# anenbergb/Co-DETR-TensorRT

Hardware: AMD Instinct MI355X
Metric: images/sec, Co-DINO Swin-L 1920x1280 fp16 (p50 ms/image alongside) (higher is better)
Workload: dtype f16

## Files before the change

co-detr-tensorrt_amd/csrc/device_prims.h:

```cpp
#pragma once
#include <hip/hip_runtime.h>
#include <stdint.h>

namespace {

typedef _Float16 f16x8 __attribute__((ext_vector_type(8)));
typedef _Float16 f16x4 __attribute__((ext_vector_type(4)));
typedef _Float16 f16x2 __attribute__((ext_vector_type(2)));
typedef __bf16 bf16x8 __attribute__((ext_vector_type(8)));
typedef __bf16 bf16x4 __attribute__((ext_vector_type(4)));
typedef __bf16 bf16x2 __attribute__((ext_vector_type(2)));
typedef short s16x8 __attribute__((ext_vector_type(8)));
typedef short s16x4 __attribute__((ext_vector_type(4)));
typedef unsigned short u16x8 __attribute__((ext_vector_type(8)));
typedef unsigned short u16x4 __attribute__((ext_vector_type(4)));
typedef unsigned short u16x2 __attribute__((ext_vector_type(2)));
typedef float f32x4 __attribute__((ext_vector_type(4)));
typedef float f32x2 __attribute__((ext_vector_type(2)));
typedef unsigned u32x4 __attribute__((ext_vector_type(4)));
typedef unsigned u32x2 __attribute__((ext_vector_type(2)));
typedef int i32x8 __attribute__((ext_vector_type(8)));
typedef int i32x4 __attribute__((ext_vector_type(4)));

__device__ __forceinline__ float bf16_to_f32(unsigned short bits) { return __uint_as_float(((unsigned)bits) << 16); }
__device__ __forceinline__ unsigned short bf16_from_f32(float v) {
  const unsigned u = __float_as_uint(v);
  if ((u & 0x7fffffffu) > 0x7f800000u) return (unsigned short)((u >> 16) | 0x40);
  return (unsigned short)((u + 0x7fffu + ((u >> 16) & 1u)) >> 16);
}

template <class F, short kNegInf>
__device__ __forceinline__ F relu_bits16(F x) {
  s16x8 i;
  __builtin_memcpy(&i, &x, 16);
  u32x4 keep = __builtin_bit_cast(u32x4, __builtin_elementwise_sub_sat((s16x8)kNegInf, i) >> 15);
  asm("" : "+v"(keep));
  i = __builtin_bit_cast(s16x8, __builtin_bit_cast(u32x4, i) & keep);
  __builtin_memcpy(&x, &i, 16);
  return x;
}

struct HalfT {
  using elem = _Float16;
  using frag = f16x8;
  using v4 = f16x4;
  __device__ static f32x4 mfma(frag a, frag b, f32x4 c) { return __builtin_amdgcn_mfma_f32_16x16x32_f16(a, b, c, 0, 0, 0); }
  __device__ static float to_f32(unsigned short bits) {
    _Float16 h;
    __builtin_memcpy(&h, &bits, 2);
    return (float)h;
  }
  __device__ static unsigned short from_f32(float v) {
    _Float16 h = (_Float16)v;
    unsigned short bits;
    __builtin_memcpy(&bits, &h, 2);
    return bits;
  }
  __device__ static unsigned pack2(float lo, float hi) {
    f16x2 h = {(_Float16)lo, (_Float16)hi};
    unsigned o;
    __builtin_memcpy(&o, &h, 4);
    return o;
  }
  __device__ static s16x4 pack4(const float (&v)[4]) {
    f16x4 h = {(_Float16)v[0], (_Float16)v[1], (_Float16)v[2], (_Float16)v[3]};
    s16x4 o;
    __builtin_memcpy(&o, &h, 8);
    return o;
  }
  __device__ static frag relu(frag x) { return relu_bits16<frag, (short)0xfc00>(x); }
};
struct BFloatT {
  using elem = __bf16;
  using frag = bf16x8;
  using v4 = bf16x4;
  __device__ static f32x4 mfma(frag a, frag b, f32x4 c) { return __builtin_amdgcn_mfma_f32_16x16x32_bf16(a, b, c, 0, 0, 0); }
  __device__ static float to_f32(unsigned short bits) { return bf16_to_f32(bits); }
  __device__ static unsigned short from_f32(float v) {
    const __bf16 h = (__bf16)v;
    return __builtin_bit_cast(unsigned short, h);
  }
  __device__ static unsigned pack2(float lo, float hi) {
    const bf16x2 h = {(__bf16)lo, (__bf16)hi};
    return __builtin_bit_cast(unsigned, h);
  }
  __device__ static s16x4 pack4(const float (&v)[4]) {
    const bf16x4 h = {(__bf16)v[0], (__bf16)v[1], (__bf16)v[2], (__bf16)v[3]};
    return __builtin_bit_cast(s16x4, h);
  }
  __device__ static frag relu(frag x) { return relu_bits16<frag, (short)0xff80>(x); }
};

__device__ __forceinline__ float gelu_erf(float x) {
  const float u = fabsf(x);
  const float t = __builtin_amdgcn_rcpf(fmaf(0.3275911f * 0.70710678118654752f, u, 1.0f));
  float p = fmaf(0.5f * 1.061405429f, t, 0.5f * -1.453152027f);
  p = fmaf(p, t, 0.5f * 1.421413741f);
  p = fmaf(p, t, 0.5f * -0.284496736f);
  p = fmaf(p, t, 0.5f * 0.254829592f);
  const float ez = __builtin_amdgcn_exp2f(u * u * (-0.5f * 1.4426950408889634f));
  return fmaf(u, fmaf(-(p * t), ez, 0.5f), 0.5f * x);
}
__device__ __forceinline__ f32x2 gelu_erf2(f32x2 x) {
  const f32x2 u = {fabsf(x.x), fabsf(x.y)};
  const f32x2 d = __builtin_elementwise_fma(f32x2{0.3275911f * 0.70710678118654752f, 0.3275911f * 0.70710678118654752f}, u,
                                            f32x2{1.0f, 1.0f});
  const f32x2 t = {__builtin_amdgcn_rcpf(d.x), __builtin_amdgcn_rcpf(d.y)};
  f32x2 p = __builtin_elementwise_fma(f32x2{0.5f * 1.061405429f, 0.5f * 1.061405429f}, t,
                                      f32x2{0.5f * -1.453152027f, 0.5f * -1.453152027f});
  p = __builtin_elementwise_fma(p, t, f32x2{0.5f * 1.421413741f, 0.5f * 1.421413741f});
  p = __builtin_elementwise_fma(p, t, f32x2{0.5f * -0.284496736f, 0.5f * -0.284496736f});
  p = __builtin_elementwise_fma(p, t, f32x2{0.5f * 0.254829592f, 0.5f * 0.254829592f});
  const f32x2 e = (u * u) * f32x2{-0.5f * 1.4426950408889634f, -0.5f * 1.4426950408889634f};
  const f32x2 ez = {__builtin_amdgcn_exp2f(e.x), __builtin_amdgcn_exp2f(e.y)};
  const f32x2 h = __builtin_elementwise_fma(-(p * t), ez, f32x2{0.5f, 0.5f});
  return __builtin_elementwise_fma(u, h, x * f32x2{0.5f, 0.5f});
}

__device__ __forceinline__ unsigned xcd_tile(unsigned bid, unsigned nblk) {
  const unsigned q = nblk >> 3, r = nblk & 7u, x = bid & 7u, i = bid >> 3;
  return (x < r ? x * (q + 1) : r * (q + 1) + (x - r) * q) + i;
}

__device__ __forceinline__ void lds_dma16(const unsigned char* src, unsigned voff, unsigned lds_addr) {
  asm volatile("s_mov_b32 m0, %2\n\ts_nop 0\n\tglobal_load_lds_dwordx4 %0, %1" ::"v"(voff), "s"(src), "s"(lds_addr)
               : "memory", "m0");
}
__device__ __forceinline__ void lds_dma16(const unsigned char* src, unsigned voff, unsigned char* dst) {
  lds_dma16(src, voff, (unsigned)(uintptr_t)((__attribute__((address_space(3))) unsigned char*)dst));
}
__device__ __forceinline__ void lds_dma16_auto(const void* g, unsigned char* l) {
  __builtin_amdgcn_global_load_lds((const __attribute__((address_space(1))) void*)g,
                                   (__attribute__((address_space(3))) void*)l, 16, 0, 0);
}
template <int N>
__device__ __forceinline__ void wait_vmcnt() {
  asm volatile("s_waitcnt vmcnt(%0)" ::"n"(N) : "memory");
}

__device__ __forceinline__ int floor_i(float v) {
  int d;
  asm("v_cvt_flr_i32_f32 %0, %1" : "=v"(d) : "v"(v));
  return d;
}

template <int CTRL>
__device__ __forceinline__ unsigned dpp_u(unsigned v) {
  return (unsigned)__builtin_amdgcn_update_dpp(0, (int)v, CTRL, 0xf, 0xf, true);
}
template <int CTRL>
__device__ __forceinline__ float dpp_f(float v) {
  return __uint_as_float(dpp_u<CTRL>(__float_as_uint(v)));
}
constexpr int kXor1 = 0xB1, kXor2 = 0x4E;
__device__ __forceinline__ unsigned quad_bcast_u(unsigned v, int owner) {
  switch (owner) {
    case 0: return dpp_u<0x00>(v);
    case 1: return dpp_u<0x55>(v);
    case 2: return dpp_u<0xAA>(v);
    default: return dpp_u<0xFF>(v);
  }
}
__device__ __forceinline__ float quad_bcast_f(float v, int owner) { return __uint_as_float(quad_bcast_u(__float_as_uint(v), owner)); }
__device__ __forceinline__ unsigned quad_bcast_add(unsigned v, int owner, unsigned add) {
  unsigned d;
  switch (owner) {
    case 0: asm("v_add_u32_dpp %0, %1, %2 quad_perm:[0,0,0,0] row_mask:0xf bank_mask:0xf" : "=v"(d) : "v"(v), "v"(add)); break;
    case 1: asm("v_add_u32_dpp %0, %1, %2 quad_perm:[1,1,1,1] row_mask:0xf bank_mask:0xf" : "=v"(d) : "v"(v), "v"(add)); break;
    case 2: asm("v_add_u32_dpp %0, %1, %2 quad_perm:[2,2,2,2] row_mask:0xf bank_mask:0xf" : "=v"(d) : "v"(v), "v"(add)); break;
    default: asm("v_add_u32_dpp %0, %1, %2 quad_perm:[3,3,3,3] row_mask:0xf bank_mask:0xf" : "=v"(d) : "v"(v), "v"(add)); break;
  }
  return d;
}

}
```

co-detr-tensorrt_amd/csrc/ffn_fused.hip:

```cpp
#include <hip/hip_runtime.h>
#include <stdint.h>

#include <type_traits>

#include "codetr_hip.h"
#include "device_prims.h"
#include "large_lds.h"

#ifdef CODETR_FFN_ABL
#define CODETR_FFN_ABL_MASK CODETR_FFN_ABL
#else
#define CODETR_FFN_ABL_MASK 0
#endif
namespace {

constexpr int C = 256;
constexpr int BH = 64;
constexpr int kThreads = 256;
constexpr int kW1Bytes = BH * C * 2;
constexpr int kW2Bytes = C * BH * 2;
constexpr int kStageBytes = kW1Bytes + kW2Bytes;
constexpr int kMaxHidden = 8192;


template <class ET, int MTT = 2, bool OPROJ = false>
__global__ __launch_bounds__(kThreads) __attribute__((amdgpu_waves_per_eu(1, 1))) void ffn_fused_kernel(
    const unsigned short* __restrict__ X, const unsigned short* __restrict__ W1, const unsigned short* __restrict__ b1,
    const unsigned short* __restrict__ W2, const unsigned short* __restrict__ b2, unsigned short* __restrict__ Y, int M,
    int Hd, const unsigned short* __restrict__ ln_g, const unsigned short* __restrict__ ln_b, float ln_eps,
    const unsigned short* __restrict__ pos, unsigned short* __restrict__ Y2,
    const unsigned short* __restrict__ lnin_g, const unsigned short* __restrict__ lnin_b, float lnin_eps, int ntiles,
    const unsigned short* __restrict__ Wo = nullptr, const unsigned short* __restrict__ bo = nullptr,
    const unsigned short* __restrict__ ID = nullptr) {
  __shared__ __attribute__((aligned(16))) unsigned char lds[2 * kStageBytes + kMaxHidden * 2 + 2048];
  using E = typename ET::elem;
  using V8 = typename ET::frag;
  using V4 = typename ET::v4;
  constexpr int MT = MTT, WR = 16 * MT, TR = 4 * WR;
  const int tid = threadIdx.x, lane = tid & 63;
  const int wave = __builtin_amdgcn_readfirstlane(tid >> 6);
  const int l15 = lane & 15, grp = lane >> 4;
  const int nchunks = Hd / BH;
  unsigned char* ringA = lds;
  unsigned char* ringB = lds + 2 * kW1Bytes;
  unsigned short* sB1 = reinterpret_cast<unsigned short*>(lds + 2 * kStageBytes);
  unsigned short* sLn = reinterpret_cast<unsigned short*>(lds + 2 * kStageBytes + kMaxHidden * 2);
  unsigned short* sB2 = sLn + 512;
  unsigned short* sBo = sB2 + 256;

  unsigned w1_voff[2];
#pragma unroll
  for (int par = 0; par < 2; ++par)
    w1_voff[par] = (unsigned)((tid >> 5) * (C * 2) + (((tid & 31) ^ ((par * 8 + (tid >> 5)) & 15)) * 16));
  const unsigned w2_voff = (unsigned)((tid >> 3) * Hd * 2 + (((tid & 7) ^ ((tid >> 4) & 7)) * 16));
  const unsigned char* W1b = reinterpret_cast<const unsigned char*>(W1);
  const unsigned char* W2b = reinterpret_cast<const unsigned char*>(W2);
  const unsigned char* Wob = reinterpret_cast<const unsigned char*>(Wo);
  auto stage_w1 = [&](int p, int c, unsigned char* dst) {
    lds_dma16(W1b + (size_t)c * kW1Bytes + p * 4096, w1_voff[p & 1], dst + (p * kThreads + wave * 64) * 16);
  };
  auto stage_wo = [&](int p, int c, unsigned char* dst) {
    lds_dma16(Wob + (size_t)c * kW1Bytes + p * 4096, w1_voff[p & 1], dst + (p * kThreads + wave * 64) * 16);
  };
  auto stage_w2 = [&](int q, int c, unsigned char* dst) {
    lds_dma16(W2b + (size_t)q * 64 * Hd + c * (BH * 2), w2_voff, dst + (q * kThreads + wave * 64) * 16);
  };
#pragma unroll
  for (int p = 0; p < 8; ++p) {
    if (OPROJ) stage_wo(p, 0, ringA);
    else stage_w1(p, 0, ringA);
  }
#pragma unroll
  for (int p = 0; p < 8; ++p) stage_w2(p, 0, ringB);
  if (OPROJ) {
#pragma unroll
    for (int p = 0; p < 8; ++p) stage_wo(p, 1, ringA + kW1Bytes);
  }

  V8 xn[MT][8];
  auto load_x = [&](int tile, int mt) {
    int m = tile * TR + wave * WR + mt * 16 + l15;
    m = m < M ? m : M - 1;
#pragma unroll
    for (int ks = 0; ks < 8; ++ks) xn[mt][ks] = *reinterpret_cast<const V8*>(X + (size_t)m * C + ks * 32 + grp * 8);
  };
#pragma unroll
  for (int mt = 0; mt < MT; ++mt) load_x(blockIdx.x, mt);
  for (int i = tid; i < Hd / 8; i += kThreads)
    *reinterpret_cast<s16x8*>(sB1 + i * 8) = *reinterpret_cast<const s16x8*>(b1 + i * 8);
  if (ln_g && tid < 64) {
    const int i = tid & 31;
    *reinterpret_cast<s16x8*>(sLn + (tid >> 5) * 256 + i * 8) = *reinterpret_cast<const s16x8*>((tid >> 5 ? ln_b : ln_g) + i * 8);
  }
  if (tid >= 64 && tid < 96) *reinterpret_cast<s16x8*>(sB2 + (tid - 64) * 8) = *reinterpret_cast<const s16x8*>(b2 + (tid - 64) * 8);
  if (OPROJ && tid >= 96 && tid < 128) *reinterpret_cast<s16x8*>(sBo + (tid - 96) * 8) = *reinterpret_cast<const s16x8*>(bo + (tid - 96) * 8);
  asm volatile("s_waitcnt lgkmcnt(0)" ::: "memory");

  int gc = 0;
  int ga = 0;
  for (int tile = blockIdx.x; tile < ntiles; tile += gridDim.x) {
    const int m0 = tile * TR + wave * WR;
    V8 xf[MT][8];
    f32x4 yacc[16][MT];
    if constexpr (OPROJ) {
      const int cb = 16 * (grp & 1) + 8 * (grp >> 1);
      V8 idn[MT][8];
#pragma unroll
      for (int mt = 0; mt < MT; ++mt) {
        int m = m0 + mt * 16 + l15;
        m = m < M ? m : M - 1;
#pragma unroll
        for (int j = 0; j < 8; ++j) {
          if (CODETR_FFN_ABL_MASK & 32) idn[mt][j] = xn[mt][j];
          else idn[mt][j] = *reinterpret_cast<const V8*>(ID + (size_t)m * C + 32 * j + cb);
        }
      }
#pragma unroll
      for (int mt = 0; mt < MT; ++mt) asm volatile("" ::"v"(xn[mt][7]) : "memory");
#pragma unroll
      for (int nt = 0; nt < 16; ++nt)
#pragma unroll
        for (int mt = 0; mt < MT; ++mt) yacc[nt][mt] = f32x4{0.f, 0.f, 0.f, 0.f};
      unsigned char* const A0 = ringA + (ga & 1) * kW1Bytes;
      unsigned char* const A1 = ringA + ((ga + 1) & 1) * kW1Bytes;
      unsigned char* const B1 = ringB + ((gc + 1) & 1) * kW2Bytes;
#pragma unroll
      for (int pc = 0; pc < 4; ++pc) {
        const unsigned char* sW = pc == 0 ? A0 : pc == 1 ? A1 : pc == 2 ? B1 : A0;
        if (pc >= 2 && !(CODETR_FFN_ABL_MASK & 256)) wait_vmcnt<8>();
        __builtin_amdgcn_s_barrier();
        auto read_wo = [&](int ks, V8 (&a)[4]) {
#pragma unroll
          for (int ht = 0; ht < 4; ++ht) {
            const int row = ht * 16 + l15;
            const int chunk = (ks * 4 + grp) ^ (row & 15);
            a[ht] = *reinterpret_cast<const V8*>(sW + row * (C * 2) + chunk * 16);
          }
        };
        V8 aw[2][4];
        read_wo(0, aw[0]);
#pragma unroll
        for (int ks = 0; ks < 8; ++ks) {
          if (ks + 1 < 8) read_wo(ks + 1, aw[(ks + 1) & 1]);
          if (pc == 0 && !(CODETR_FFN_ABL_MASK & 256)) stage_wo(ks, 2, B1);
          else if (pc == 1 && !(CODETR_FFN_ABL_MASK & 256)) stage_wo(ks, 3, A0);
          else if (pc == 2) stage_w1(ks, 0, A1);
#pragma unroll
          for (int i = 0; i < 4 * MT; ++i)
            if (!(CODETR_FFN_ABL_MASK & 128))
              yacc[4 * pc + i / MT][i % MT] = ET::mfma(aw[ks & 1][i / MT], xn[i % MT][ks], yacc[4 * pc + i / MT][i % MT]);
            else asm volatile("" ::"v"(aw[ks & 1][i / MT]));
          __builtin_amdgcn_sched_group_barrier(0x008, 2, 0);
          __builtin_amdgcn_sched_group_barrier(0x100, 4, 0);
          __builtin_amdgcn_sched_group_barrier(0x008, 4 * MT - 2, 0);
          __builtin_amdgcn_sched_barrier(0);
        }
      }
      ga += 3;
      const int oddp = grp & 1;
      if (CODETR_FFN_ABL_MASK & 64) {
#pragma unroll
        for (int mt = 0; mt < MT; ++mt)
#pragma unroll
          for (int j = 0; j < 8; ++j) {
            xf[mt][j] = xn[mt][j];
            asm volatile("" ::"v"(idn[mt][j]), "v"(yacc[2 * j][mt]), "v"(yacc[2 * j + 1][mt]));
          }
      } else
#pragma unroll
      for (int mt = 0; mt < MT; ++mt) {
        unsigned yp[16][2];
#pragma unroll
        for (int nt = 0; nt < 16; ++nt) {
          const V4 bb = *reinterpret_cast<const V4*>(sBo + nt * 16 + grp * 4);
          const V4 y = {(E)(yacc[nt][mt][0] + (float)bb[0]), (E)(yacc[nt][mt][1] + (float)bb[1]),
                        (E)(yacc[nt][mt][2] + (float)bb[2]), (E)(yacc[nt][mt][3] + (float)bb[3])};
          __builtin_memcpy(yp[nt], &y, 8);
        }
        float o[8][8];
        float sm = 0.f;
#pragma unroll
        for (int j = 0; j < 8; ++j) {
          const unsigned s0 = oddp ? yp[2 * j][0] : yp[2 * j + 1][0], s1 = oddp ? yp[2 * j][1] : yp[2 * j + 1][1];
          const unsigned k0 = oddp ? yp[2 * j + 1][0] : yp[2 * j][0], k1 = oddp ? yp[2 * j + 1][1] : yp[2 * j][1];
          const unsigned r0 = (unsigned)__shfl_xor((int)s0, 16, 64), r1 = (unsigned)__shfl_xor((int)s1, 16, 64);
          const unsigned z[4] = {oddp ? r0 : k0, oddp ? r1 : k1, oddp ? k0 : r0, oddp ? k1 : r1};
          V8 yv;
          __builtin_memcpy(&yv, z, 16);
#pragma unroll
          for (int e = 0; e < 8; ++e) {
            o[j][e] = (float)(E)((float)yv[e] + (float)idn[mt][j][e]);
            sm += o[j][e];
          }
        }
        if (lnin_g) {
          sm += __shfl_xor(sm, 16, 64);
          sm += __shfl_xor(sm, 32, 64);
          const float mean = sm * (1.0f / C);
          float q = 0.f;
#pragma unroll
          for (int j = 0; j < 8; ++j)
#pragma unroll
            for (int e = 0; e < 8; ++e) {
              const float d = o[j][e] - mean;
              q = fmaf(d, d, q);
            }
          q += __shfl_xor(q, 16, 64);
          q += __shfl_xor(q, 32, 64);
          const float rstd = rsqrtf(q * (1.0f / C) + lnin_eps);
#pragma unroll
          for (int j = 0; j < 8; ++j) {
            const V8 gw = *reinterpret_cast<const V8*>(lnin_g + 32 * j + cb);
            const V8 gb = *reinterpret_cast<const V8*>(lnin_b + 32 * j + cb);
#pragma unroll
            for (int e = 0; e < 8; ++e) o[j][e] = fmaf((o[j][e] - mean) * rstd, (float)gw[e], (float)gb[e]);
          }
        }
#pragma unroll
        for (int j = 0; j < 8; ++j)
#pragma unroll
          for (int e = 0; e < 8; ++e) xf[mt][j][e] = (E)o[j][e];
      }
    } else {
#pragma unroll
    for (int mt = 0; mt < MT; ++mt) {
      if (lnin_g) {
        float sm = 0.f;
#pragma unroll
        for (int ks = 0; ks < 8; ++ks)
#pragma unroll
          for (int e = 0; e < 8; ++e) sm += (float)xn[mt][ks][e];
        sm += __shfl_xor(sm, 16, 64);
        sm += __shfl_xor(sm, 32, 64);
        const float mean = sm * (1.0f / C);
        float q = 0.f;
#pragma unroll
        for (int ks = 0; ks < 8; ++ks)
#pragma unroll
          for (int e = 0; e < 8; ++e) {
            const float d = (float)xn[mt][ks][e] - mean;
            q = fmaf(d, d, q);
          }
        q += __shfl_xor(q, 16, 64);
        q += __shfl_xor(q, 32, 64);
        const float rstd = rsqrtf(q * (1.0f / C) + lnin_eps);
#pragma unroll
        for (int ks = 0; ks < 8; ++ks) {
          const V8 gw = *reinterpret_cast<const V8*>(lnin_g + ks * 32 + grp * 8);
          const V8 gb = *reinterpret_cast<const V8*>(lnin_b + ks * 32 + grp * 8);
#pragma unroll
          for (int e = 0; e < 8; ++e)
            xf[mt][ks][e] = (E)fmaf(((float)xn[mt][ks][e] - mean) * rstd, (float)gw[e], (float)gb[e]);
        }
      } else {
#pragma unroll
        for (int ks = 0; ks < 8; ++ks) xf[mt][ks] = xn[mt][ks];
      }
      asm volatile("" ::"v"(xn[mt][7]) : "memory");
    }
    }
#pragma unroll
    for (int nt = 0; nt < 16; ++nt)
#pragma unroll
      for (int mt = 0; mt < MT; ++mt) yacc[nt][mt] = f32x4{0.f, 0.f, 0.f, 0.f};

    for (int c = 0; c < nchunks; ++c, ++gc, ++ga) {
      const int cn = c + 1 < nchunks ? c + 1 : 0;
      const unsigned char* sW1 = ringA + (ga & 1) * kW1Bytes;
      const unsigned char* sW2 = ringB + (gc & 1) * kW2Bytes;
      unsigned char* nW1 = ringA + ((ga + 1) & 1) * kW1Bytes;
      unsigned char* nW2 = ringB + ((gc + 1) & 1) * kW2Bytes;
      const unsigned char* nsrc1 = (OPROJ && c + 1 == nchunks) ? Wob : W1b + (size_t)cn * kW1Bytes;
      if (!(CODETR_FFN_ABL_MASK & 8)) {
        if (c > 0) wait_vmcnt<8>();
        else if (OPROJ) wait_vmcnt<0>();
        __builtin_amdgcn_s_barrier();
      }

      f32x4 hacc[4][MT];
#pragma unroll
      for (int ht = 0; ht < 4; ++ht) {
        const V4 bv = *reinterpret_cast<const V4*>(sB1 + c * BH + ht * 16 + grp * 4);
        const f32x4 b4 = {(float)bv[0], (float)bv[1], (float)bv[2], (float)bv[3]};
#pragma unroll
        for (int mt = 0; mt < MT; ++mt) hacc[ht][mt] = b4;
      }
      auto read_w1 = [&](int ks, V8 (&a)[4]) {
#pragma unroll
        for (int ht = 0; ht < 4; ++ht) {
          const int row = ht * 16 + l15;
          const int chunk = (ks * 4 + grp) ^ (row & 15);
          a[ht] = *reinterpret_cast<const V8*>(sW1 + row * (C * 2) + chunk * 16);
        }
      };
      V8 aw[2][4];
      read_w1(0, aw[0]);
#pragma unroll
      for (int ks = 0; ks < 8; ++ks) {
        if (ks + 1 < 8 && !(CODETR_FFN_ABL_MASK & 4)) read_w1(ks + 1, aw[(ks + 1) & 1]);
        if (!(CODETR_FFN_ABL_MASK & 1)) lds_dma16(nsrc1 + ks * 4096, w1_voff[ks & 1], nW1 + (ks * kThreads + wave * 64) * 16);
#pragma unroll
        for (int i = 0; i < 4 * MT; ++i)
          if (!(CODETR_FFN_ABL_MASK & 2))
            hacc[i / MT][i % MT] = ET::mfma(aw[(CODETR_FFN_ABL_MASK & 4) ? 0 : (ks & 1)][i / MT], xf[i % MT][ks], hacc[i / MT][i % MT]);
          else if (!(CODETR_FFN_ABL_MASK & 4)) asm volatile("" ::"v"(aw[ks & 1][i / MT]));
        __builtin_amdgcn_sched_group_barrier(0x008, 2, 0);
        __builtin_amdgcn_sched_group_barrier(0x100, 4, 0);
        __builtin_amdgcn_sched_group_barrier(0x008, 4 * MT - 2, 0);
        __builtin_amdgcn_sched_barrier(0);
      }
      V8 pf[2][MT];
      if (CODETR_FFN_ABL_MASK & 16) {
#pragma unroll
        for (int s = 0; s < 2; ++s)
#pragma unroll
          for (int mt = 0; mt < MT; ++mt) pf[s][mt] = xf[mt][s];
#pragma unroll
        for (int ht = 0; ht < 4; ++ht)
#pragma unroll
          for (int mt = 0; mt < MT; ++mt) asm volatile("" ::"v"(hacc[ht][mt]));
      } else
#pragma unroll
      for (int s = 0; s < 2; ++s)
#pragma unroll
        for (int mt = 0; mt < MT; ++mt)
#pragma unroll
          for (int h = 0; h < 2; ++h)
#pragma unroll
            for (int r = 0; r < 4; ++r) pf[s][mt][h * 4 + r] = (E)hacc[2 * s + h][mt][r];
      if (!(CODETR_FFN_ABL_MASK & 16))
#pragma unroll
      for (int s = 0; s < 2; ++s)
#pragma unroll
        for (int mt = 0; mt < MT; ++mt) pf[s][mt] = ET::relu(pf[s][mt]);
      if (!(CODETR_FFN_ABL_MASK & 8)) {
        if (c > 0) wait_vmcnt<8>();
        __builtin_amdgcn_s_barrier();
      }
      auto read_w2 = [&](int ntp, V8 (&a)[4]) {
#pragma unroll
        for (int t = 0; t < 2; ++t) {
          const int n = (2 * ntp + t) * 16 + l15;
          const unsigned char* rowp = sW2 + n * (BH * 2);
          const int sw = (n >> 1) & 7;
#pragma unroll
          for (int s = 0; s < 2; ++s) a[t * 2 + s] = *reinterpret_cast<const V8*>(rowp + ((4 * s + grp) ^ sw) * 16);
        }
      };
      V8 a2[2][4];
      read_w2(0, a2[0]);
#pragma unroll
      for (int ntp = 0; ntp < 8; ++ntp) {
        if (ntp + 1 < 8 && !(CODETR_FFN_ABL_MASK & 4)) read_w2(ntp + 1, a2[(ntp + 1) & 1]);
        if (!(CODETR_FFN_ABL_MASK & 1)) stage_w2(ntp, cn, nW2);
#pragma unroll
        for (int i = 0; i < 4 * MT; ++i) {
          const int ts = i / MT, mt = i % MT, nt = 2 * ntp + ts / 2;
          if (!(CODETR_FFN_ABL_MASK & 2))
            yacc[nt][mt] = ET::mfma(a2[(CODETR_FFN_ABL_MASK & 4) ? 0 : (ntp & 1)][ts], pf[ts & 1][mt], yacc[nt][mt]);
          else if (!(CODETR_FFN_ABL_MASK & 4)) asm volatile("" ::"v"(a2[ntp & 1][ts]));
        }
        __builtin_amdgcn_sched_group_barrier(0x008, 2, 0);
        __builtin_amdgcn_sched_group_barrier(0x100, 4, 0);
        __builtin_amdgcn_sched_group_barrier(0x008, 4 * MT - 2, 0);
        __builtin_amdgcn_sched_barrier(0);
      }
    }

    const int next_tile = tile + (int)gridDim.x < ntiles ? tile + (int)gridDim.x : tile;
    if (OPROJ) {
#pragma unroll
      for (int p = 0; p < 8; ++p) stage_wo(p, 1, ringA + ((ga + 1) & 1) * kW1Bytes);
    }
    const int odd = grp & 1;
    const int cbase = 16 * odd + 8 * (grp >> 1);
    const int src_lane4 = (l15 + 16 * (2 * odd + (grp >> 1))) * 4;
#pragma unroll
    for (int mt = 0; mt < MT; ++mt) {
      const int m = m0 + mt * 16 + l15;
      if (MT == 2 && mt == 0) load_x(next_tile, 0);
      unsigned yp[16][2];
#pragma unroll
      for (int nt = 0; nt < 16; ++nt) {
        const V4 bb = *reinterpret_cast<const V4*>(sB2 + nt * 16 + grp * 4);
        const V4 y = {(E)(yacc[nt][mt][0] + (float)bb[0]), (E)(yacc[nt][mt][1] + (float)bb[1]),
                      (E)(yacc[nt][mt][2] + (float)bb[2]), (E)(yacc[nt][mt][3] + (float)bb[3])};
        __builtin_memcpy(yp[nt], &y, 8);
      }
      float o[8][8];
      float sm = 0.f;
#pragma unroll
      for (int j = 0; j < 8; ++j) {
        const unsigned s0 = odd ? yp[2 * j][0] : yp[2 * j + 1][0], s1 = odd ? yp[2 * j][1] : yp[2 * j + 1][1];
        const unsigned k0 = odd ? yp[2 * j + 1][0] : yp[2 * j][0], k1 = odd ? yp[2 * j + 1][1] : yp[2 * j][1];
        const unsigned r0 = (unsigned)__shfl_xor((int)s0, 16, 64), r1 = (unsigned)__shfl_xor((int)s1, 16, 64);
        const unsigned z[4] = {odd ? r0 : k0, odd ? r1 : k1, odd ? k0 : r0, odd ? k1 : r1};
        V8 yv, xid;
        __builtin_memcpy(&yv, z, 16);
        int xw[4];
        __builtin_memcpy(xw, &xf[mt][j], 16);
        if (!OPROJ)
#pragma unroll
        for (int d = 0; d < 4; ++d) xw[d] = __builtin_amdgcn_ds_bpermute(src_lane4, xw[d]);
        __builtin_memcpy(&xid, xw, 16);
#pragma unroll
        for (int e = 0; e < 8; ++e) {
          o[j][e] = (float)(E)((float)yv[e] + (float)xid[e]);
          sm += o[j][e];
        }
      }
      V8 pr[8];
      if (Y2) {
        const unsigned short* prow = pos + (size_t)(m < M ? m : M - 1) * C + cbase;
#pragma unroll
        for (int j = 0; j < 8; ++j) pr[j] = *reinterpret_cast<const V8*>(prow + 32 * j);
      }
      if (mt == 0) load_x(next_tile, MT - 1);
      if (ln_g) {
        sm += __shfl_xor(sm, 16, 64);
        sm += __shfl_xor(sm, 32, 64);
        const float mean = sm * (1.0f / C);
        float q = 0.f;
#pragma unroll
        for (int j = 0; j < 8; ++j)
#pragma unroll
          for (int e = 0; e < 8; ++e) {
            const float d = o[j][e] - mean;
            q = fmaf(d, d, q);
          }
        q += __shfl_xor(q, 16, 64);
        q += __shfl_xor(q, 32, 64);
        const float rstd = rsqrtf(q * (1.0f / C) + ln_eps);
#pragma unroll
        for (int j = 0; j < 8; ++j) {
          const V8 gw = *reinterpret_cast<const V8*>(sLn + 32 * j + cbase);
          const V8 gb = *reinterpret_cast<const V8*>(sLn + 256 + 32 * j + cbase);
#pragma unroll
          for (int e = 0; e < 8; ++e) o[j][e] = (float)(E)fmaf((o[j][e] - mean) * rstd, (float)gw[e], (float)gb[e]);
        }
      }
      if (m < M) {
        unsigned short* yrow = Y + (size_t)m * C + cbase;
#pragma unroll
        for (int j = 0; j < 8; ++j) {
          V8 ov;
#pragma unroll
          for (int e = 0; e < 8; ++e) ov[e] = (E)o[j][e];
          *reinterpret_cast<V8*>(yrow + 32 * j) = ov;
        }
        if (Y2) {
          unsigned short* y2row = Y2 + (size_t)m * C + cbase;
#pragma unroll
          for (int j = 0; j < 8; ++j) {
            V8 ov;
#pragma unroll
            for (int e = 0; e < 8; ++e) ov[e] = (E)(o[j][e] + (float)pr[j][e]);
            *reinterpret_cast<V8*>(y2row + 32 * j) = ov;
          }
        }
      }
    }
  }
  wait_vmcnt<0>();
}

__global__ void pack_w2_kernel(const unsigned short* __restrict__ w2, unsigned short* __restrict__ out, int64_t total) {
  const int64_t i = (int64_t)blockIdx.x * blockDim.x + threadIdx.x;
  if (i >= total) return;
  const int col = (int)(i & 63);
  const int s = col >> 5, g = (col >> 3) & 3, j = col & 7;
  const int old = 32 * s + (j < 4 ? 4 * g + j : 16 + 4 * g + (j - 4));
  out[i] = w2[(i & ~(int64_t)63) + old];
}

}

namespace {

template <class ET>
int ffn_entry(void* stream, const void* x_dev, const void* w1_dev, const void* b1_dev,
                            const void* w2_packed_dev, const void* b2_dev, void* y_dev, int64_t M, int64_t C_in,
                            int64_t hidden, const void* ln_in_gamma_dev, const void* ln_in_beta_dev, float ln_in_eps,
                            const void* ln_gamma_dev, const void* ln_beta_dev, float ln_eps, const void* pos_dev,
                            void* y_plus_pos_dev, const void* wo_dev = nullptr, const void* bo_dev = nullptr,
                            const void* identity_dev = nullptr) {
  const void* w2_dev = w2_packed_dev;
  if (!x_dev || !w1_dev || !b1_dev || !w2_dev || !b2_dev || !y_dev || M <= 0 || hidden <= 0) return CODETR_E_BADARG;
  const bool oproj = wo_dev != nullptr;
  if (oproj && (!bo_dev || !identity_dev)) return CODETR_E_BADARG;
  if ((reinterpret_cast<uintptr_t>(wo_dev) | reinterpret_cast<uintptr_t>(bo_dev) | reinterpret_cast<uintptr_t>(identity_dev)) & 15)
    return CODETR_E_BADARG;
  if ((ln_gamma_dev == nullptr) != (ln_beta_dev == nullptr) || (pos_dev == nullptr) != (y_plus_pos_dev == nullptr) ||
      (ln_in_gamma_dev == nullptr) != (ln_in_beta_dev == nullptr))
    return CODETR_E_BADARG;
  if (C_in != C || hidden % BH != 0 || hidden > kMaxHidden) return CODETR_E_UNSUPPORTED;
  if (M > 0x7fffffffLL - 256 || hidden > 0x7fffffffLL) return CODETR_E_TOO_LARGE;
  if ((reinterpret_cast<uintptr_t>(x_dev) | reinterpret_cast<uintptr_t>(w1_dev) | reinterpret_cast<uintptr_t>(b1_dev) |
       reinterpret_cast<uintptr_t>(w2_dev) | reinterpret_cast<uintptr_t>(b2_dev) | reinterpret_cast<uintptr_t>(y_dev) |
       reinterpret_cast<uintptr_t>(ln_in_gamma_dev) | reinterpret_cast<uintptr_t>(ln_in_beta_dev) |
       reinterpret_cast<uintptr_t>(ln_gamma_dev) | reinterpret_cast<uintptr_t>(ln_beta_dev) |
       reinterpret_cast<uintptr_t>(pos_dev) | reinterpret_cast<uintptr_t>(y_plus_pos_dev)) & 15)
    return CODETR_E_BADARG;
  const int cus = device_cus();
  const int64_t ntiles_all = (M + 127) / 128;
  const int64_t left = ntiles_all % cus;
  const bool split = left > 0 && 2 * left <= cus;
  const int64_t M1 = split ? (ntiles_all - left) * 128 : M;
  auto launch = [&](auto mt_tag, int64_t row0, int64_t rows) {
    constexpr int MTT = decltype(mt_tag)::value;
    const int ntiles = (int)((rows + 64 * MTT - 1) / (64 * MTT));
    const unsigned blocks = (unsigned)(ntiles < cus ? ntiles : cus);
    const size_t off = (size_t)row0 * C;
    auto at = [&](const void* p) { return p ? static_cast<const unsigned short*>(p) + off : nullptr; };
#define CODETR_FFN_ARGS \
    at(x_dev), static_cast<const unsigned short*>(w1_dev), static_cast<const unsigned short*>(b1_dev), \
        static_cast<const unsigned short*>(w2_dev), static_cast<const unsigned short*>(b2_dev), \
        const_cast<unsigned short*>(at(y_dev)), (int)rows, (int)hidden, static_cast<const unsigned short*>(ln_gamma_dev), \
        static_cast<const unsigned short*>(ln_beta_dev), ln_eps, at(pos_dev), const_cast<unsigned short*>(at(y_plus_pos_dev)), \
        static_cast<const unsigned short*>(ln_in_gamma_dev), static_cast<const unsigned short*>(ln_in_beta_dev), ln_in_eps, ntiles
    if (oproj)
      hipLaunchKernelGGL((ffn_fused_kernel<ET, MTT, true>), dim3(blocks), dim3(kThreads), 0, static_cast<hipStream_t>(stream),
                         CODETR_FFN_ARGS, static_cast<const unsigned short*>(wo_dev),
                         static_cast<const unsigned short*>(bo_dev), at(identity_dev));
    else
      hipLaunchKernelGGL((ffn_fused_kernel<ET, MTT, false>), dim3(blocks), dim3(kThreads), 0, static_cast<hipStream_t>(stream),
                         CODETR_FFN_ARGS);
#undef CODETR_FFN_ARGS
  };
  if (M1 > 0) launch(std::integral_constant<int, 2>{}, 0, M1);
  if (split) launch(std::integral_constant<int, 1>{}, M1, M - M1);
  const hipError_t err = hipGetLastError();
  return err == hipSuccess ? 0 : (int)err;
}

}

extern "C" {

int codetr_ffn_pack_w2_f16(void* stream, const void* w2_dev, void* w2_packed_dev, int64_t C_out, int64_t hidden) {
  if (!w2_dev || !w2_packed_dev || C_out <= 0 || hidden <= 0) return CODETR_E_BADARG;
  if (hidden % BH != 0) return CODETR_E_UNSUPPORTED;
  const int64_t total = C_out * hidden;
  hipLaunchKernelGGL(pack_w2_kernel, dim3((unsigned)((total + 255) / 256)), dim3(256), 0, static_cast<hipStream_t>(stream),
                     static_cast<const unsigned short*>(w2_dev), static_cast<unsigned short*>(w2_packed_dev), total);
  const hipError_t err = hipGetLastError();
  return err == hipSuccess ? 0 : (int)err;
}

int codetr_ffn_relu_ln2_f16(void* stream, const void* x_dev, const void* w1_dev, const void* b1_dev,
                            const void* w2_packed_dev, const void* b2_dev, void* y_dev, int64_t M, int64_t C_in,
                            int64_t hidden, const void* ln_in_gamma_dev, const void* ln_in_beta_dev, float ln_in_eps,
                            const void* ln_gamma_dev, const void* ln_beta_dev, float ln_eps, const void* pos_dev,
                            void* y_plus_pos_dev) {
  return ffn_entry<HalfT>(stream, x_dev, w1_dev, b1_dev, w2_packed_dev, b2_dev, y_dev, M, C_in, hidden, ln_in_gamma_dev,
                         ln_in_beta_dev, ln_in_eps, ln_gamma_dev, ln_beta_dev, ln_eps, pos_dev, y_plus_pos_dev);
}

int codetr_ffn_relu_ln2_bf16(void* stream, const void* x_dev, const void* w1_dev, const void* b1_dev,
                            const void* w2_packed_dev, const void* b2_dev, void* y_dev, int64_t M, int64_t C_in,
                            int64_t hidden, const void* ln_in_gamma_dev, const void* ln_in_beta_dev, float ln_in_eps,
                            const void* ln_gamma_dev, const void* ln_beta_dev, float ln_eps, const void* pos_dev,
                            void* y_plus_pos_dev) {
  return ffn_entry<BFloatT>(stream, x_dev, w1_dev, b1_dev, w2_packed_dev, b2_dev, y_dev, M, C_in, hidden, ln_in_gamma_dev,
                         ln_in_beta_dev, ln_in_eps, ln_gamma_dev, ln_beta_dev, ln_eps, pos_dev, y_plus_pos_dev);
}

int codetr_ffn_oproj_relu_ln2_f16(void* stream, const void* attn_dev, const void* wo_dev, const void* bo_dev,
                                  const void* identity_dev, const void* w1_perm_dev, const void* b1_dev,
                                  const void* w2_packed_dev, const void* b2_dev, void* y_dev, int64_t M, int64_t C_in,
                                  int64_t hidden, const void* ln_in_gamma_dev, const void* ln_in_beta_dev, float ln_in_eps,
                                  const void* ln_gamma_dev, const void* ln_beta_dev, float ln_eps, const void* pos_dev,
                                  void* y_plus_pos_dev) {
  if (!wo_dev) return CODETR_E_BADARG;
  return ffn_entry<HalfT>(stream, attn_dev, w1_perm_dev, b1_dev, w2_packed_dev, b2_dev, y_dev, M, C_in, hidden, ln_in_gamma_dev,
                         ln_in_beta_dev, ln_in_eps, ln_gamma_dev, ln_beta_dev, ln_eps, pos_dev, y_plus_pos_dev, wo_dev, bo_dev,
                         identity_dev);
}

int codetr_ffn_oproj_relu_ln2_bf16(void* stream, const void* attn_dev, const void* wo_dev, const void* bo_dev,
                                   const void* identity_dev, const void* w1_perm_dev, const void* b1_dev,
                                   const void* w2_packed_dev, const void* b2_dev, void* y_dev, int64_t M, int64_t C_in,
                                   int64_t hidden, const void* ln_in_gamma_dev, const void* ln_in_beta_dev, float ln_in_eps,
                                   const void* ln_gamma_dev, const void* ln_beta_dev, float ln_eps, const void* pos_dev,
                                   void* y_plus_pos_dev) {
  if (!wo_dev) return CODETR_E_BADARG;
  return ffn_entry<BFloatT>(stream, attn_dev, w1_perm_dev, b1_dev, w2_packed_dev, b2_dev, y_dev, M, C_in, hidden,
                          ln_in_gamma_dev, ln_in_beta_dev, ln_in_eps, ln_gamma_dev, ln_beta_dev, ln_eps, pos_dev,
                          y_plus_pos_dev, wo_dev, bo_dev, identity_dev);
}

int codetr_ffn_oproj_w1_index(int64_t C_in, int32_t* idx_host) {
  if (!idx_host || C_in != C) return CODETR_E_BADARG;
  for (int s = 0; s < C / 32; ++s)
    for (int g = 0; g < 4; ++g)
      for (int e = 0; e < 8; ++e) idx_host[32 * s + 8 * g + e] = 32 * s + 16 * (g & 1) + 8 * (g >> 1) + e;
  return 0;
}

int codetr_ffn_relu_ln_f16(void* stream, const void* x_dev, const void* w1_dev, const void* b1_dev,
                           const void* w2_packed_dev, const void* b2_dev, void* y_dev, int64_t M, int64_t C_in,
                           int64_t hidden, const void* ln_gamma_dev, const void* ln_beta_dev, float ln_eps,
                           const void* pos_dev, void* y_plus_pos_dev) {
  return codetr_ffn_relu_ln2_f16(stream, x_dev, w1_dev, b1_dev, w2_packed_dev, b2_dev, y_dev, M, C_in, hidden, nullptr,
                                 nullptr, 0.f, ln_gamma_dev, ln_beta_dev, ln_eps, pos_dev, y_plus_pos_dev);
}

int codetr_ffn_relu_f16(void* stream, const void* x_dev, const void* w1_dev, const void* b1_dev,
                        const void* w2_packed_dev, const void* b2_dev, void* y_dev, int64_t M, int64_t C_in,
                        int64_t hidden) {
  return codetr_ffn_relu_ln_f16(stream, x_dev, w1_dev, b1_dev, w2_packed_dev, b2_dev, y_dev, M, C_in, hidden, nullptr,
                                nullptr, 0.f, nullptr, nullptr);
}

}
```

Before: 97.90.

## Streamline FFN epilogue with permlane swaps, packed math and fp32 param tables

Reworks the fused FFN kernel epilogues. Cross-row exchange now uses permlane16 swaps instead of conditional shfl_xor selects, and row reductions use permlane16/32 swaps. Biases and LayerNorm parameters are preconverted into LDS tables (fp32 for biases, native or fp32 for norm params), and residual adds and packing use packed vector ops. Input-LN parameters are staged in LDS instead of read from global memory, at the cost of a larger LDS footprint and an extra barrier. Optional cycle-stamp instrumentation is added behind a compile flag.

```diff
diff --git a/co-detr-tensorrt_amd/csrc/device_prims.h b/co-detr-tensorrt_amd/csrc/device_prims.h
--- a/co-detr-tensorrt_amd/csrc/device_prims.h
+++ b/co-detr-tensorrt_amd/csrc/device_prims.h
@@ -69,6 +69,24 @@
     return o;
   }
   __device__ static frag relu(frag x) { return relu_bits16<frag, (short)0xfc00>(x); }
+  __device__ static frag add8(frag a, frag b) {
+    frag s = a + b;
+    asm("" : "+v"(s));
+    return s;
+  }
+  using param = _Float16;
+  __device__ static param to_param(unsigned short bits) { return __builtin_bit_cast(_Float16, bits); }
+  __device__ static frag norm8(const float (&d)[8], float rstd, const param* g, const param* b) {
+    const frag gw = *reinterpret_cast<const frag*>(g), gb = *reinterpret_cast<const frag*>(b);
+    frag o;
+#pragma unroll
+    for (int e = 0; e < 8; e += 2) {
+      const f32x2 t = f32x2{d[e], d[e + 1]} * f32x2{rstd, rstd};
+      o[e] = (_Float16)fmaf(t.x, (float)gw[e], (float)gb[e]);
+      o[e + 1] = (_Float16)fmaf(t.y, (float)gw[e + 1], (float)gb[e + 1]);
+    }
+    return o;
+  }
 };
 struct BFloatT {
   using elem = __bf16;
@@ -89,7 +107,46 @@
     return __builtin_bit_cast(s16x4, h);
   }
   __device__ static frag relu(frag x) { return relu_bits16<frag, (short)0xff80>(x); }
+  __device__ static frag add8(frag a, frag b) {
+    const u32x4 ua = __builtin_bit_cast(u32x4, a), ub = __builtin_bit_cast(u32x4, b);
+    u32x4 o;
+#pragma unroll
+    for (int d = 0; d < 4; ++d) {
+      const f32x2 s = f32x2{__uint_as_float(ua[d] << 16), __uint_as_float(ua[d] & 0xffff0000u)} +
+                      f32x2{__uint_as_float(ub[d] << 16), __uint_as_float(ub[d] & 0xffff0000u)};
+      o[d] = pack2(s.x, s.y);
+    }
+    return __builtin_bit_cast(frag, o);
+  }
+  using param = float;
+  __device__ static param to_param(unsigned short bits) { return bf16_to_f32(bits); }
+  __device__ static frag norm8(const float (&d)[8], float rstd, const param* g, const param* b) {
+    const f32x4 g0 = *reinterpret_cast<const f32x4*>(g), g1 = *reinterpret_cast<const f32x4*>(g + 4);
+    const f32x4 b0 = *reinterpret_cast<const f32x4*>(b), b1 = *reinterpret_cast<const f32x4*>(b + 4);
+    const float gw[8] = {g0[0], g0[1], g0[2], g0[3], g1[0], g1[1], g1[2], g1[3]};
+    const float gb[8] = {b0[0], b0[1], b0[2], b0[3], b1[0], b1[1], b1[2], b1[3]};
+    u32x4 o;
+#pragma unroll
+    for (int e = 0; e < 8; e += 2) {
+      const f32x2 t = f32x2{d[e], d[e + 1]} * f32x2{rstd, rstd};
+      const f32x2 r = __builtin_elementwise_fma(t, f32x2{gw[e], gw[e + 1]}, f32x2{gb[e], gb[e + 1]});
+      o[e / 2] = pack2(r.x, r.y);
+    }
+    return __builtin_bit_cast(frag, o);
+  }
 };
+
+template <class ET>
+__device__ __forceinline__ u32x2 bias_pack4(f32x4 acc, f32x4 bias) {
+  const f32x2 lo = f32x2{acc[0], acc[1]} + f32x2{bias[0], bias[1]};
+  const f32x2 hi = f32x2{acc[2], acc[3]} + f32x2{bias[2], bias[3]};
+  return u32x2{ET::pack2(lo.x, lo.y), ET::pack2(hi.x, hi.y)};
+}
+template <class ET>
+__device__ __forceinline__ typename ET::frag pack8(const float (&v)[8]) {
+  const u32x4 o = {ET::pack2(v[0], v[1]), ET::pack2(v[2], v[3]), ET::pack2(v[4], v[5]), ET::pack2(v[6], v[7])};
+  return __builtin_bit_cast(typename ET::frag, o);
+}
 
 __device__ __forceinline__ float gelu_erf(float x) {
   const float u = fabsf(x);
@@ -144,6 +201,19 @@
   return d;
 }
 
+__device__ __forceinline__ void swap_rows16(unsigned& a, unsigned& b) {
+  const auto r = __builtin_amdgcn_permlane16_swap(a, b, false, false);
+  a = r[0], b = r[1];
+}
+__device__ __forceinline__ float add_xor16(float v) {
+  const auto r = __builtin_amdgcn_permlane16_swap(__float_as_uint(v), __float_as_uint(v), false, false);
+  return __uint_as_float(r[0]) + __uint_as_float(r[1]);
+}
+__device__ __forceinline__ float add_xor32(float v) {
+  const auto r = __builtin_amdgcn_permlane32_swap(__float_as_uint(v), __float_as_uint(v), false, false);
+  return __uint_as_float(r[0]) + __uint_as_float(r[1]);
+}
+
 template <int CTRL>
 __device__ __forceinline__ unsigned dpp_u(unsigned v) {
   return (unsigned)__builtin_amdgcn_update_dpp(0, (int)v, CTRL, 0xf, 0xf, true);
diff --git a/co-detr-tensorrt_amd/csrc/ffn_fused.hip b/co-detr-tensorrt_amd/csrc/ffn_fused.hip
--- a/co-detr-tensorrt_amd/csrc/ffn_fused.hip
+++ b/co-detr-tensorrt_amd/csrc/ffn_fused.hip
@@ -13,6 +13,18 @@
 #define CODETR_FFN_ABL_MASK 0
 #endif
 namespace {
+
+#ifdef CODETR_FFN_STAMPS
+__device__ unsigned long long* g_ffn_stamps = nullptr;
+#define FFN_T(i)                            \
+  __builtin_amdgcn_sched_barrier(0);        \
+  const unsigned long long ffn_t##i = __builtin_readcyclecounter(); \
+  __builtin_amdgcn_sched_barrier(0)
+#define FFN_ACC(k, a, b) ffn_acc[k] += ffn_t##b - ffn_t##a
+#else
+#define FFN_T(i)
+#define FFN_ACC(k, a, b)
+#endif
 
 constexpr int C = 256;
 constexpr int BH = 64;
@@ -21,7 +33,25 @@
 constexpr int kW2Bytes = C * BH * 2;
 constexpr int kStageBytes = kW1Bytes + kW2Bytes;
 constexpr int kMaxHidden = 8192;
-
+constexpr int kTableBytes = 2 * C * 4 + 2 * (2 * C * 4);
+
+
+__device__ __forceinline__ float row_stats(float (&o)[8][8], float sm, float eps) {
+  sm = add_xor32(add_xor16(sm));
+  const float mean = sm * (1.0f / C);
+  float q = 0.f;
+#pragma unroll
+  for (int j = 0; j < 8; ++j)
+#pragma unroll
+    for (int e = 0; e < 8; e += 2) {
+      const f32x2 d = f32x2{o[j][e], o[j][e + 1]} - f32x2{mean, mean};
+      o[j][e] = d.x, o[j][e + 1] = d.y;
+      q = fmaf(d.x, d.x, q);
+      q = fmaf(d.y, d.y, q);
+    }
+  q = add_xor32(add_xor16(q));
+  return rsqrtf(q * (1.0f / C) + eps);
+}
 
 template <class ET, int MTT = 2, bool OPROJ = false>
 __global__ __launch_bounds__(kThreads) __attribute__((amdgpu_waves_per_eu(1, 1))) void ffn_fused_kernel(
@@ -32,10 +62,11 @@
     const unsigned short* __restrict__ lnin_g, const unsigned short* __restrict__ lnin_b, float lnin_eps, int ntiles,
     const unsigned short* __restrict__ Wo = nullptr, const unsigned short* __restrict__ bo = nullptr,
     const unsigned short* __restrict__ ID = nullptr) {
-  __shared__ __attribute__((aligned(16))) unsigned char lds[2 * kStageBytes + kMaxHidden * 2 + 2048];
+  __shared__ __attribute__((aligned(16))) unsigned char lds[2 * kStageBytes + kMaxHidden * 2 + kTableBytes];
   using E = typename ET::elem;
   using V8 = typename ET::frag;
   using V4 = typename ET::v4;
+  using P = typename ET::param;
   constexpr int MT = MTT, WR = 16 * MT, TR = 4 * WR;
   const int tid = threadIdx.x, lane = tid & 63;
   const int wave = __builtin_amdgcn_readfirstlane(tid >> 6);
@@ -44,9 +75,10 @@
   unsigned char* ringA = lds;
   unsigned char* ringB = lds + 2 * kW1Bytes;
   unsigned short* sB1 = reinterpret_cast<unsigned short*>(lds + 2 * kStageBytes);
-  unsigned short* sLn = reinterpret_cast<unsigned short*>(lds + 2 * kStageBytes + kMaxHidden * 2);
-  unsigned short* sB2 = sLn + 512;
-  unsigned short* sBo = sB2 + 256;
+  float* sB2 = reinterpret_cast<float*>(lds + 2 * kStageBytes + kMaxHidden * 2);
+  float* sBo = sB2 + C;
+  P* sLn = reinterpret_cast<P*>(sBo + C);
+  P* sLnIn = reinterpret_cast<P*>(reinterpret_cast<float*>(sLn) + 2 * C);
 
   unsigned w1_voff[2];
 #pragma unroll
@@ -88,18 +120,29 @@
   for (int mt = 0; mt < MT; ++mt) load_x(blockIdx.x, mt);
   for (int i = tid; i < Hd / 8; i += kThreads)
     *reinterpret_cast<s16x8*>(sB1 + i * 8) = *reinterpret_cast<const s16x8*>(b1 + i * 8);
-  if (ln_g && tid < 64) {
-    const int i = tid & 31;
-    *reinterpret_cast<s16x8*>(sLn + (tid >> 5) * 256 + i * 8) = *reinterpret_cast<const s16x8*>((tid >> 5 ? ln_b : ln_g) + i * 8);
+  static_assert(kThreads == C, "one thread per channel");
+  sB2[tid] = ET::to_f32(b2[tid]);
+  if (OPROJ) sBo[tid] = ET::to_f32(bo[tid]);
+  if (ln_g) {
+    sLn[tid] = ET::to_param(ln_g[tid]);
+    sLn[C + tid] = ET::to_param(ln_b[tid]);
   }
-  if (tid >= 64 && tid < 96) *reinterpret_cast<s16x8*>(sB2 + (tid - 64) * 8) = *reinterpret_cast<const s16x8*>(b2 + (tid - 64) * 8);
-  if (OPROJ && tid >= 96 && tid < 128) *reinterpret_cast<s16x8*>(sBo + (tid - 96) * 8) = *reinterpret_cast<const s16x8*>(bo + (tid - 96) * 8);
+  if (lnin_g) {
+    sLnIn[tid] = ET::to_param(lnin_g[tid]);
+    sLnIn[C + tid] = ET::to_param(lnin_b[tid]);
+  }
   asm volatile("s_waitcnt lgkmcnt(0)" ::: "memory");
-
+  if (!OPROJ) __builtin_amdgcn_s_barrier();
+
+#ifdef CODETR_FFN_STAMPS
+  unsigned long long ffn_acc[5] = {0, 0, 0, 0, 0};
+  const unsigned long long ffn_k0 = __builtin_readcyclecounter();
+#endif
   int gc = 0;
   int ga = 0;
   for (int tile = blockIdx.x; tile < ntiles; tile += gridDim.x) {
     const int m0 = tile * TR + wave * WR;
+    FFN_T(0);
     V8 xf[MT][8];
     f32x4 yacc[16][MT];
     if constexpr (OPROJ) {
@@ -157,7 +200,9 @@
         }
       }
       ga += 3;
-      const int oddp = grp & 1;
+      FFN_T(1);
+      FFN_ACC(0, 0, 1);
+      FFN_ACC(1, 1, 0);
       if (CODETR_FFN_ABL_MASK & 64) {
 #pragma unroll
         for (int mt = 0; mt < MT; ++mt)
@@ -172,86 +217,51 @@
         unsigned yp[16][2];
 #pragma unroll
         for (int nt = 0; nt < 16; ++nt) {
-          const V4 bb = *reinterpret_cast<const V4*>(sBo + nt * 16 + grp * 4);
-          const V4 y = {(E)(yacc[nt][mt][0] + (float)bb[0]), (E)(yacc[nt][mt][1] + (float)bb[1]),
-                        (E)(yacc[nt][mt][2] + (float)bb[2]), (E)(yacc[nt][mt][3] + (float)bb[3])};
-          __builtin_memcpy(yp[nt], &y, 8);
+          const u32x2 y = bias_pack4<ET>(yacc[nt][mt], *reinterpret_cast<const f32x4*>(sBo + nt * 16 + grp * 4));
+          yp[nt][0] = y[0], yp[nt][1] = y[1];
         }
         float o[8][8];
         float sm = 0.f;
 #pragma unroll
         for (int j = 0; j < 8; ++j) {
-          const unsigned s0 = oddp ? yp[2 * j][0] : yp[2 * j + 1][0], s1 = oddp ? yp[2 * j][1] : yp[2 * j + 1][1];
-          const unsigned k0 = oddp ? yp[2 * j + 1][0] : yp[2 * j][0], k1 = oddp ? yp[2 * j + 1][1] : yp[2 * j][1];
-          const unsigned r0 = (unsigned)__shfl_xor((int)s0, 16, 64), r1 = (unsigned)__shfl_xor((int)s1, 16, 64);
-          const unsigned z[4] = {oddp ? r0 : k0, oddp ? r1 : k1, oddp ? k0 : r0, oddp ? k1 : r1};
+          swap_rows16(yp[2 * j][0], yp[2 * j + 1][0]);
+          swap_rows16(yp[2 * j][1], yp[2 * j + 1][1]);
+          const unsigned z[4] = {yp[2 * j][0], yp[2 * j][1], yp[2 * j + 1][0], yp[2 * j + 1][1]};
           V8 yv;
           __builtin_memcpy(&yv, z, 16);
+          const V8 ev = ET::add8(yv, idn[mt][j]);
 #pragma unroll
           for (int e = 0; e < 8; ++e) {
-            o[j][e] = (float)(E)((float)yv[e] + (float)idn[mt][j][e]);
+            o[j][e] = (float)ev[e];
             sm += o[j][e];
           }
         }
         if (lnin_g) {
-          sm += __shfl_xor(sm, 16, 64);
-          sm += __shfl_xor(sm, 32, 64);
-          const float mean = sm * (1.0f / C);
-          float q = 0.f;
-#pragma unroll
-          for (int j = 0; j < 8; ++j)
-#pragma unroll
-            for (int e = 0; e < 8; ++e) {
-              const float d = o[j][e] - mean;
-              q = fmaf(d, d, q);
-            }
-          q += __shfl_xor(q, 16, 64);
-          q += __shfl_xor(q, 32, 64);
-          const float rstd = rsqrtf(q * (1.0f / C) + lnin_eps);
-#pragma unroll
-          for (int j = 0; j < 8; ++j) {
-            const V8 gw = *reinterpret_cast<const V8*>(lnin_g + 32 * j + cb);
-            const V8 gb = *reinterpret_cast<const V8*>(lnin_b + 32 * j + cb);
-#pragma unroll
-            for (int e = 0; e < 8; ++e) o[j][e] = fmaf((o[j][e] - mean) * rstd, (float)gw[e], (float)gb[e]);
-          }
-        }
-#pragma unroll
-        for (int j = 0; j < 8; ++j)
-#pragma unroll
-          for (int e = 0; e < 8; ++e) xf[mt][j][e] = (E)o[j][e];
+          const float rstd = row_stats(o, sm, lnin_eps);
+#pragma unroll
+          for (int j = 0; j < 8; ++j) xf[mt][j] = ET::norm8(o[j], rstd, sLnIn + 32 * j + cb, sLnIn + C + 32 * j + cb);
+        } else {
+#pragma unroll
+          for (int j = 0; j < 8; ++j) xf[mt][j] = pack8<ET>(o[j]);
+        }
       }
     } else {
 #pragma unroll
     for (int mt = 0; mt < MT; ++mt) {
       if (lnin_g) {
+        float o[8][8];
         float sm = 0.f;
 #pragma unroll
         for (int ks = 0; ks < 8; ++ks)
 #pragma unroll
-          for (int e = 0; e < 8; ++e) sm += (float)xn[mt][ks][e];
-        sm += __shfl_xor(sm, 16, 64);
-        sm += __shfl_xor(sm, 32, 64);
-        const float mean = sm * (1.0f / C);
-        float q = 0.f;
+          for (int e = 0; e < 8; ++e) {
+            o[ks][e] = (float)xn[mt][ks][e];
+            sm += o[ks][e];
+          }
+        const float rstd = row_stats(o, sm, lnin_eps);
 #pragma unroll
         for (int ks = 0; ks < 8; ++ks)
-#pragma unroll
-          for (int e = 0; e < 8; ++e) {
-            const float d = (float)xn[mt][ks][e] - mean;
-            q = fmaf(d, d, q);
-          }
-        q += __shfl_xor(q, 16, 64);
-        q += __shfl_xor(q, 32, 64);
-        const float rstd = rsqrtf(q * (1.0f / C) + lnin_eps);
-#pragma unroll
-        for (int ks = 0; ks < 8; ++ks) {
-          const V8 gw = *reinterpret_cast<const V8*>(lnin_g + ks * 32 + grp * 8);
-          const V8 gb = *reinterpret_cast<const V8*>(lnin_b + ks * 32 + grp * 8);
-#pragma unroll
-          for (int e = 0; e < 8; ++e)
-            xf[mt][ks][e] = (E)fmaf(((float)xn[mt][ks][e] - mean) * rstd, (float)gw[e], (float)gb[e]);
-        }
+          xf[mt][ks] = ET::norm8(o[ks], rstd, sLnIn + ks * 32 + grp * 8, sLnIn + C + ks * 32 + grp * 8);
       } else {
 #pragma unroll
         for (int ks = 0; ks < 8; ++ks) xf[mt][ks] = xn[mt][ks];
@@ -259,6 +269,8 @@
       asm volatile("" ::"v"(xn[mt][7]) : "memory");
     }
     }
+    FFN_T(2);
+    FFN_ACC(1, 0, 2);
 #pragma unroll
     for (int nt = 0; nt < 16; ++nt)
 #pragma unroll
@@ -367,6 +379,8 @@
       }
     }
 
+    FFN_T(3);
+    FFN_ACC(2, 2, 3);
     const int next_tile = tile + (int)gridDim.x < ntiles ? tile + (int)gridDim.x : tile;
     if (OPROJ) {
 #pragma unroll
@@ -382,19 +396,16 @@
       unsigned yp[16][2];
 #pragma unroll
       for (int nt = 0; nt < 16; ++nt) {
-        const V4 bb = *reinterpret_cast<const V4*>(sB2 + nt * 16 + grp * 4);
-        const V4 y = {(E)(yacc[nt][mt][0] + (float)bb[0]), (E)(yacc[nt][mt][1] + (float)bb[1]),
-                      (E)(yacc[nt][mt][2] + (float)bb[2]), (E)(yacc[nt][mt][3] + (float)bb[3])};
-        __builtin_memcpy(yp[nt], &y, 8);
+        const u32x2 y = bias_pack4<ET>(yacc[nt][mt], *reinterpret_cast<const f32x4*>(sB2 + nt * 16 + grp * 4));
+        yp[nt][0] = y[0], yp[nt][1] = y[1];
       }
       float o[8][8];
       float sm = 0.f;
 #pragma unroll
       for (int j = 0; j < 8; ++j) {
-        const unsigned s0 = odd ? yp[2 * j][0] : yp[2 * j + 1][0], s1 = odd ? yp[2 * j][1] : yp[2 * j + 1][1];
-        const unsigned k0 = odd ? yp[2 * j + 1][0] : yp[2 * j][0], k1 = odd ? yp[2 * j + 1][1] : yp[2 * j][1];
-        const unsigned r0 = (unsigned)__shfl_xor((int)s0, 16, 64), r1 = (unsigned)__shfl_xor((int)s1, 16, 64);
-        const unsigned z[4] = {odd ? r0 : k0, odd ? r1 : k1, odd ? k0 : r0, odd ? k1 : r1};
+        swap_rows16(yp[2 * j][0], yp[2 * j + 1][0]);
+        swap_rows16(yp[2 * j][1], yp[2 * j + 1][1]);
+        const unsigned z[4] = {yp[2 * j][0], yp[2 * j][1], yp[2 * j + 1][0], yp[2 * j + 1][1]};
         V8 yv, xid;
         __builtin_memcpy(&yv, z, 16);
         int xw[4];
@@ -403,9 +414,10 @@
 #pragma unroll
         for (int d = 0; d < 4; ++d) xw[d] = __builtin_amdgcn_ds_bpermute(src_lane4, xw[d]);
         __builtin_memcpy(&xid, xw, 16);
+        const V8 ev = ET::add8(yv, xid);
 #pragma unroll
         for (int e = 0; e < 8; ++e) {
-          o[j][e] = (float)(E)((float)yv[e] + (float)xid[e]);
+          o[j][e] = (float)ev[e];
           sm += o[j][e];
         }
       }
@@ -416,52 +428,40 @@
         for (int j = 0; j < 8; ++j) pr[j] = *reinterpret_cast<const V8*>(prow + 32 * j);
       }
       if (mt == 0) load_x(next_tile, MT - 1);
+      V8 ov[8];
       if (ln_g) {
-        sm += __shfl_xor(sm, 16, 64);
-        sm += __shfl_xor(sm, 32, 64);
-        const float mean = sm * (1.0f / C);
-        float q = 0.f;
-#pragma unroll
-        for (int j = 0; j < 8; ++j)
-#pragma unroll
-          for (int e = 0; e < 8; ++e) {
-            const float d = o[j][e] - mean;
-            q = fmaf(d, d, q);
-          }
-        q += __shfl_xor(q, 16, 64);
-        q += __shfl_xor(q, 32, 64);
-        const float rstd = rsqrtf(q * (1.0f / C) + ln_eps);
-#pragma unroll
-        for (int j = 0; j < 8; ++j) {
-          const V8 gw = *reinterpret_cast<const V8*>(sLn + 32 * j + cbase);
-          const V8 gb = *reinterpret_cast<const V8*>(sLn + 256 + 32 * j + cbase);
-#pragma unroll
-          for (int e = 0; e < 8; ++e) o[j][e] = (float)(E)fmaf((o[j][e] - mean) * rstd, (float)gw[e], (float)gb[e]);
-        }
+        const float rstd = row_stats(o, sm, ln_eps);
+#pragma unroll
+        for (int j = 0; j < 8; ++j) ov[j] = ET::norm8(o[j], rstd, sLn + 32 * j + cbase, sLn + C + 32 * j + cbase);
+      } else {
+#pragma unroll
+        for (int j = 0; j < 8; ++j) ov[j] = pack8<ET>(o[j]);
       }
       if (m < M) {
         unsigned short* yrow = Y + (size_t)m * C + cbase;
 #pragma unroll
-        for (int j = 0; j < 8; ++j) {
-          V8 ov;
-#pragma unroll
-          for (int e = 0; e < 8; ++e) ov[e] = (E)o[j][e];
-          *reinterpret_cast<V8*>(yrow + 32 * j) = ov;
-        }
+        for (int j = 0; j < 8; ++j) *reinterpret_cast<V8*>(yrow + 32 * j) = ov[j];
         if (Y2) {
           unsigned short* y2row = Y2 + (size_t)m * C + cbase;
 #pragma unroll
-          for (int j = 0; j < 8; ++j) {
-            V8 ov;
-#pragma unroll
-            for (int e = 0; e < 8; ++e) ov[e] = (E)(o[j][e] + (float)pr[j][e]);
-            *reinterpret_cast<V8*>(y2row + 32 * j) = ov;
-          }
+          for (int j = 0; j < 8; ++j) *reinterpret_cast<V8*>(y2row + 32 * j) = ET::add8(ov[j], pr[j]);
         }
       }
     }
+    FFN_T(4);
+    FFN_ACC(3, 3, 4);
+#ifdef CODETR_FFN_STAMPS
+    ffn_acc[4] += 1;
+#endif
   }
   wait_vmcnt<0>();
+#ifdef CODETR_FFN_STAMPS
+  if (lane == 0 && g_ffn_stamps) {
+    unsigned long long* o = g_ffn_stamps + ((size_t)blockIdx.x * 4 + wave) * 8;
+    for (int i = 0; i < 5; ++i) o[i] = ffn_acc[i];
+    o[5] = __builtin_readcyclecounter() - ffn_k0;
+  }
+#endif
 }
 
 __global__ void pack_w2_kernel(const unsigned short* __restrict__ w2, unsigned short* __restrict__ out, int64_t total) {
```

Result: no change. 98.52, median of 6 (+0.6%).
